# zfkuang/PaletteNeRF

Measured on AMD Instinct MI355X. Metric: rendered_samples_per_sec, higher is better.
Workload: dtype f32 (field: f16x3 split products, fp32 accumulate); 1 GPU; configs[1]: NeRF-synthetic lego geometry (scene S0), -m nerf inference, 800x800, 1 view(s)/step, camera moving (one pose of the path per step); march_mode=native, fused_field=True, field_precision=f16x3, half_tables=False, ray_order=tile8, frames_in_flight=1, gathered_floats_per_ray=0, rccl_ranks=1, parallelism=single GPU

## Files before the change

palettenerf_amd/csrc/field_core.hpp:

```cpp
#pragma once
#include "pnr_common.hpp"
#include "sh_eval.hpp"

namespace pnr {

typedef float f32x16 __attribute__((ext_vector_type(16)));

constexpr int kS0 = 0;
constexpr int kS1 = kS0 + 2 * 16 * 64;
constexpr int kC0 = kS1 + 1 * 32 * 64;
constexpr int kC1 = kC0 + 2 * 16 * 64;
constexpr int kC2 = kC1 + 2 * 32 * 64;
constexpr int kPackedFloats = kC2 + 1 * 32 * 64;

__host__ __device__ constexpr int frag_row(int r, int h) { return (r & 3) + 8 * (r >> 2) + 4 * h; }

__device__ __forceinline__ float select_half(int h, float lower, float upper) {
    const uint32_t m = 0u - (uint32_t)h;
    return __uint_as_float((__float_as_uint(lower) & ~m) | (__float_as_uint(upper) & m));
}

__device__ __forceinline__ f32x16 zero16() {
    f32x16 z;
#pragma unroll
// ... 32 lines not shown
    u32x4 hw, lw;
#pragma unroll
    for (int j = 0; j < 8; j += 2) {
        const h2v hp = {(_Float16)v[j], (_Float16)v[j + 1]};
        const uint32_t hb = __builtin_bit_cast(uint32_t, hp);
        uint32_t lb;
        asm("v_fma_mixlo_f16 %0, %1, -1.0, %2 op_sel_hi:[1,0,0]" : "=v"(lb) : "v"(hb), "v"(v[j]));
        asm("v_fma_mixhi_f16 %0, %1, -1.0, %2 op_sel:[1,0,0] op_sel_hi:[1,0,0]" : "+v"(lb) : "v"(hb), "v"(v[j + 1]));
        hw[j / 2] = hb; lw[j / 2] = lb;
    }
    asm volatile("s_nop 3" : "+v"(lw));
    hi = __builtin_bit_cast(h8, hw);
    lo = __builtin_bit_cast(h8, lw);
}
__device__ __forceinline__ void split_frag(const f32x16& a, int half_idx, h8& hi, h8& lo) {
    float v[8];
#pragma unroll
    for (int j = 0; j < 8; j++) v[j] = a[half_idx * 8 + j];
    split8(v, hi, lo);
}
constexpr int kF16MaxBits = 0x477FE000;
template <bool CHECK> struct SplitWatch;
template <> struct SplitWatch<false> {
    __device__ __forceinline__ void see(const float*) {}
    __device__ __forceinline__ bool overflowed() const { return false; }
};
template <> struct SplitWatch<true> {
    int mx = 0;
    __device__ __forceinline__ void see(const float v[8]) {
#pragma unroll
        for (int j = 0; j < 8; j += 2) mx = max(max(mx, __float_as_int(v[j]) & 0x7fffffff), __float_as_int(v[j + 1]) & 0x7fffffff);
    }
    __device__ __forceinline__ bool overflowed() const { return mx > kF16MaxBits; }
};
template <bool CHECK>
__device__ __forceinline__ void split_frag_w(SplitWatch<CHECK>& sw, const f32x16& a, int half_idx, h8& hi, h8& lo) {
    float v[8];
#pragma unroll
    for (int j = 0; j < 8; j++) v[j] = a[half_idx * 8 + j];
    sw.see(v);
    split8(v, hi, lo);
}

__device__ __forceinline__ f32x16 mma3(f32x16 acc, const unsigned char* __restrict__ wblock, const h8& bhi, const h8& blo, int lane) {
    const h8 ahi = *reinterpret_cast<const h8*>(wblock + lane * 16);
    const h8 alo = *reinterpret_cast<const h8*>(wblock + 1024 + lane * 16);
    acc = __builtin_amdgcn_mfma_f32_32x32x16_f16(alo, bhi, acc, 0, 0, 0);
    acc = __builtin_amdgcn_mfma_f32_32x32x16_f16(ahi, blo, acc, 0, 0, 0);
    acc = __builtin_amdgcn_mfma_f32_32x32x16_f16(ahi, bhi, acc, 0, 0, 0);
    return acc;
}

__device__ __forceinline__ void round8(const float v[8], h8& hi) {
    typedef uint32_t u32x4 __attribute__((ext_vector_type(4)));
    u32x4 hw;
#pragma unroll
    for (int j = 0; j < 8; j += 2) {
        const h2v hp = {(_Float16)v[j], (_Float16)v[j + 1]};
        hw[j / 2] = __builtin_bit_cast(uint32_t, hp);
    }
    hi = __builtin_bit_cast(h8, hw);
}
__device__ __forceinline__ f32x16 mma2(f32x16 acc, const unsigned char* __restrict__ wblock, const h8& bhi, int lane) {
    const h8 ahi = *reinterpret_cast<const h8*>(wblock + lane * 16);
    const h8 alo = *reinterpret_cast<const h8*>(wblock + 1024 + lane * 16);
    acc = __builtin_amdgcn_mfma_f32_32x32x16_f16(alo, bhi, acc, 0, 0, 0);
    acc = __builtin_amdgcn_mfma_f32_32x32x16_f16(ahi, bhi, acc, 0, 0, 0);
    return acc;
}
template <bool LO> __device__ __forceinline__ void splitx(const float v[8], h8& hi, h8& lo) {
    if constexpr (LO) split8(v, hi, lo); else round8(v, hi);
}
template <bool LO> __device__ __forceinline__ f32x16 mmax(f32x16 acc, const unsigned char* __restrict__ wblock, const h8& bhi, const h8& blo, int lane) {
    if constexpr (LO) return mma3(acc, wblock, bhi, blo, lane); else return mma2(acc, wblock, bhi, lane);
}
template <bool LO, bool CHECK>
__device__ __forceinline__ void splitx_frag_w(SplitWatch<CHECK>& sw, const f32x16& a, int half_idx, h8& hi, h8& lo) {
    float v[8];
#pragma unroll
    for (int j = 0; j < 8; j++) v[j] = a[half_idx * 8 + j];
    sw.see(v);
    splitx<LO>(v, hi, lo);
}

template <int PREC> struct BOp;
template <> struct BOp<1> { h8 hi, lo; };
template <> struct BOp<2> { h8 hi; };
template <> struct BOp<0> { float v[8]; };

template <int PREC, bool CHECK = false> __device__ __forceinline__ BOp<PREC> make_op(const float v[8], SplitWatch<CHECK>* sw = nullptr) {
    BOp<PREC> o;
    if constexpr (PREC == 1) { if constexpr (CHECK) sw->see(v); split8(v, o.hi, o.lo); }
    else if constexpr (PREC == 2) { if constexpr (CHECK) sw->see(v); round8(v, o.hi); }
    else {
#pragma unroll
        for (int j = 0; j < 8; j++) o.v[j] = v[j];
    }
    return o;
}
template <int PREC, bool CHECK = false> __device__ __forceinline__ BOp<PREC> frag_op(const f32x16& a, int half_idx, SplitWatch<CHECK>* sw = nullptr) {
    float v[8];
#pragma unroll
    for (int j = 0; j < 8; j++) v[j] = a[half_idx * 8 + j];
    return make_op<PREC, CHECK>(v, sw);
}
template <int PREC> __device__ __forceinline__ f32x16 mma_blk(f32x16 acc, const unsigned char* __restrict__ wblock, const BOp<PREC>& b, int lane) {
    if constexpr (PREC == 1) return mma3(acc, wblock, b.hi, b.lo, lane);
    else if constexpr (PREC == 2) return mma2(acc, wblock, b.hi, lane);
    else {
        const float* w = reinterpret_cast<const float*>(wblock);
#pragma unroll
        for (int j = 0; j < 8; j++) acc = __builtin_amdgcn_mfma_f32_32x32x2f32(w[j * 64 + lane], b.v[j], acc, 0, 0, 0);
        return acc;
    }
}

__device__ __forceinline__ void head3_valu(const unsigned char* __restrict__ vec, const f32x16& u0, const f32x16& u1, float out[3]) {
    typedef float f32x2v __attribute__((ext_vector_type(2)));
    typedef __attribute__((address_space(3))) f32x4 lds_f32x4;
    const lds_f32x4* wv = reinterpret_cast<const lds_f32x4*>(reinterpret_cast<uintptr_t>(vec));
    f32x2v acc[3] = {{0.0f, 0.0f}, {0.0f, 0.0f}, {0.0f, 0.0f}};
#pragma unroll
    for (int t = 0; t < 2; t++)
#pragma unroll
        for (int r4 = 0; r4 < 4; r4++) {
            const f32x16& u = t ? u1 : u0;
            f32x4 ww[3];
#pragma unroll
            for (int o = 0; o < 3; o++) ww[o] = wv[(o * 2 + t) * 4 + r4];
#pragma unroll
            for (int o = 0; o < 3; o++) acc[o] = __builtin_elementwise_fma(f32x2v{ww[o].x, ww[o].y}, f32x2v{u[4 * r4], u[4 * r4 + 1]}, acc[o]);
#pragma unroll
            for (int o = 0; o < 3; o++) acc[o] = __builtin_elementwise_fma(f32x2v{ww[o].z, ww[o].w}, f32x2v{u[4 * r4 + 2], u[4 * r4 + 3]}, acc[o]);
        }
#pragma unroll
    for (int o = 0; o < 3; o++) {
        const float p = acc[o].x + acc[o].y;
        const auto sw2 = __builtin_amdgcn_permlane32_swap(__float_as_uint(p), __float_as_uint(p), false, false);
        out[o] = __uint_as_float(sw2[0]) + __uint_as_float(sw2[1]);
    }
}

constexpr uint32_t kVecHeadHalfBytes = 3 * 2 * 16 * 4;
static __global__ void k_pack_vec_head(const float* __restrict__ w, float* __restrict__ out) {
    const int i = threadIdx.x;
    if (i >= 192) return;
    const int r = i & 15, t = (i >> 4) & 1, o = (i >> 5) % 3, h = i / 96;
    out[i] = w[o * 64 + 32 * t + frag_row(r, h)];
}


struct FieldOut { float sigma_logit, o0, o1, o2; };

__device__ __forceinline__ void load_enc_rows8(const float* __restrict__ enc, size_t level_stride, uint32_t row, bool valid, int h, float x[2][8]) {
    const f32x2* p[8];
    f32x2 v[8];
#pragma unroll
    for (int kb = 0; kb < 2; kb++)
#pragma unroll
        for (int q = 0; q < 4; q++) p[4 * kb + q] = reinterpret_cast<const f32x2*>(enc + ((size_t)(8 * kb + 4 * h + q) * level_stride + row) * 2);
    load8_fresh(p, v);
#pragma unroll
    for (int kb = 0; kb < 2; kb++)
#pragma unroll
        for (int q = 0; q < 4; q++) { x[kb][2 * q] = valid ? v[4 * kb + q].x : 0.0f; x[kb][2 * q + 1] = valid ? v[4 * kb + q].y : 0.0f; }
}
template <bool CHECK, bool LO = true>
__device__ __forceinline__ FieldOut nerf_field_tile_f16x3(const unsigned char* __restrict__ w, int lane, bool valid, const float* __restrict__ enc,
                                                          size_t level_stride, uint32_t row, float dx, float dy, float dz, float enc_scale,
                                                          SplitWatch<CHECK>& sw) {
    const int h = lane >> 5;
    h8 bh[2], bl[2];
    {
        float x[2][8];
        load_enc_rows8(enc, level_stride, row, valid, h, x);
        if (enc_scale != 1.0f) {
#pragma unroll
            for (int j = 0; j < 8; j++) { x[0][j] *= enc_scale; x[1][j] *= enc_scale; }
        }
        sw.see(x[0]); sw.see(x[1]);
        split8(x[0], bh[0], bl[0]);
        split8(x[1], bh[1], bl[1]);
    }
    f32x16 h0 = zero16(), h1 = zero16();
    h0 = mma3(h0, w + 0 * kF16BlockBytes, bh[0], bl[0], lane);
    h0 = mma3(h0, w + 1 * kF16BlockBytes, bh[1], bl[1], lane);
    h1 = mma3(h1, w + 2 * kF16BlockBytes, bh[0], bl[0], lane);
    h1 = mma3(h1, w + 3 * kF16BlockBytes, bh[1], bl[1], lane);
    __builtin_amdgcn_sched_barrier(0);
    h0 = relu16(h0); h1 = relu16(h1);

    f32x16 g = zero16();
#pragma unroll
    for (int kb = 0; kb < 4; kb++) {
        split_frag_w(sw, kb < 2 ? h0 : h1, kb & 1, bh[0], bl[0]);
        g = mma3(g, w + (4 + kb) * kF16BlockBytes, bh[0], bl[0], lane);
    }
    __builtin_amdgcn_sched_barrier(0);
    if (enc_scale != 1.0f) {
        const float inv = 1.0f / enc_scale;
#pragma unroll
        for (int r = 0; r < 8; r++) g[r] *= inv;
    }
    FieldOut out;
    out.sigma_logit = g[0];

    float sh[16];
    sh_eval<4>(dx, dy, dz, sh);
    {
        float v[8];
#pragma unroll
        for (int j = 0; j < 8; j++) v[j] = select_half(h, sh[j], sh[8 + j]);
        splitx<LO>(v, bh[0], bl[0]);
    }
    splitx_frag_w<LO>(sw, g, 0, bh[1], bl[1]);
    f32x16 c0 = zero16(), c1 = zero16();
    c0 = mmax<LO>(c0, w + 8 * kF16BlockBytes, bh[0], bl[0], lane);
    c0 = mmax<LO>(c0, w + 9 * kF16BlockBytes, bh[1], bl[1], lane);
    c1 = mmax<LO>(c1, w + 10 * kF16BlockBytes, bh[0], bl[0], lane);
    c1 = mmax<LO>(c1, w + 11 * kF16BlockBytes, bh[1], bl[1], lane);
    __builtin_amdgcn_sched_barrier(0);
    c0 = relu16(c0); c1 = relu16(c1);

    f32x16 d0 = zero16(), d1 = zero16();
#pragma unroll
    for (int kb = 0; kb < 4; kb++) {
        splitx_frag_w<LO>(sw, kb < 2 ? c0 : c1, kb & 1, bh[0], bl[0]);
        d0 = mmax<LO>(d0, w + (12 + kb) * kF16BlockBytes, bh[0], bl[0], lane);
        d1 = mmax<LO>(d1, w + (16 + kb) * kF16BlockBytes, bh[0], bl[0], lane);
    }
    __builtin_amdgcn_sched_barrier(0);
    d0 = relu16(d0); d1 = relu16(d1);

    float o[3];
    head3_valu(w + 20 * kF16BlockBytes + (uint32_t)h * kVecHeadHalfBytes, d0, d1, o);
    out.o0 = o[0]; out.o1 = o[1]; out.o2 = o[2];
    return out;
}

__device__ __forceinline__ FieldOut nerf_field_tile_f32(const float* __restrict__ w, int lane, bool valid, const float* __restrict__ enc,
                                                        size_t level_stride, uint32_t row, float dx, float dy, float dz) {
    const int h = lane >> 5;
    float x[16];
#pragma unroll
    for (int s = 0; s < 16; s++) x[s] = valid ? enc[((size_t)s * level_stride + row) * 2 + h] : 0.0f;
    f32x16 h0 = zero16(), h1 = zero16();
#pragma unroll
    for (int s = 0; s < 16; s++) {
        h0 = __builtin_amdgcn_mfma_f32_32x32x2f32(w[kS0 + s * 64 + lane], x[s], h0, 0, 0, 0);
        h1 = __builtin_amdgcn_mfma_f32_32x32x2f32(w[kS0 + (16 + s) * 64 + lane], x[s], h1, 0, 0, 0);
    }
    __builtin_amdgcn_sched_barrier(0);
    h0 = relu16(h0); h1 = relu16(h1);
    f32x16 g = zero16();
    g = mma_frag(g, &w[kS1], h0, lane);
    g = mma_frag(g, &w[kS1 + 16 * 64], h1, lane);
    FieldOut out;
    out.sigma_logit = g[0];
    float sh[16];
    sh_eval<4>(dx, dy, dz, sh);
    f32x16 c0 = zero16(), c1 = zero16();
#pragma unroll
    for (int s = 0; s < 8; s++) {
        const float b = select_half(h, sh[s], sh[8 + s]);
        c0 = __builtin_amdgcn_mfma_f32_32x32x2f32(w[kC0 + s * 64 + lane], b, c0, 0, 0, 0);
        c1 = __builtin_amdgcn_mfma_f32_32x32x2f32(w[kC0 + (16 + s) * 64 + lane], b, c1, 0, 0, 0);
    }
    __builtin_amdgcn_sched_barrier(0);
#pragma unroll
    for (int r = 0; r < 8; r++) {
        c0 = __builtin_amdgcn_mfma_f32_32x32x2f32(w[kC0 + (8 + r) * 64 + lane], g[r], c0, 0, 0, 0);
        c1 = __builtin_amdgcn_mfma_f32_32x32x2f32(w[kC0 + (24 + r) * 64 + lane], g[r], c1, 0, 0, 0);
    }
    __builtin_amdgcn_sched_barrier(0);
    c0 = relu16(c0); c1 = relu16(c1);
    f32x16 d0 = zero16(), d1 = zero16();
    d0 = mma_frag(d0, &w[kC1], c0, lane);
    d0 = mma_frag(d0, &w[kC1 + 16 * 64], c1, lane);
    d1 = mma_frag(d1, &w[kC1 + 32 * 64], c0, lane);
    d1 = mma_frag(d1, &w[kC1 + 48 * 64], c1, lane);
    d0 = relu16(d0); d1 = relu16(d1);
    f32x16 o = zero16();
    o = mma_frag(o, &w[kC2], d0, lane);
    o = mma_frag(o, &w[kC2 + 16 * 64], d1, lane);
    out.o0 = o[0]; out.o1 = o[1]; out.o2 = o[2];
    return out;
}

template <int PREC>
__device__ __forceinline__ f32x16 nerf_density_tile(const float* __restrict__ wf, int lane, bool valid, const float* __restrict__ enc, size_t level_stride,
                                                    uint32_t row, float enc_scale = 1.0f) {
    const int h = lane >> 5;
    f32x16 h0 = zero16(), h1 = zero16(), g = zero16();
    if constexpr (PREC == 0) {
        float x[16];
#pragma unroll
        for (int s = 0; s < 16; s++) x[s] = valid ? enc[((size_t)s * level_stride + row) * 2 + h] : 0.0f;
#pragma unroll
        for (int s = 0; s < 16; s++) {
            h0 = __builtin_amdgcn_mfma_f32_32x32x2f32(wf[kS0 + s * 64 + lane], x[s], h0, 0, 0, 0);
            h1 = __builtin_amdgcn_mfma_f32_32x32x2f32(wf[kS0 + (16 + s) * 64 + lane], x[s], h1, 0, 0, 0);
        }
        __builtin_amdgcn_sched_barrier(0);
        h0 = relu16(h0); h1 = relu16(h1);
        g = mma_frag(g, &wf[kS1], h0, lane);
        g = mma_frag(g, &wf[kS1 + 16 * 64], h1, lane);
    } else {
        const unsigned char* w = reinterpret_cast<const unsigned char*>(wf);
        h8 bh[4], bl[4];
        float x[2][8];
        load_enc_rows8(enc, level_stride, row, valid, h, x);
        if (enc_scale != 1.0f) {
#pragma unroll
            for (int j = 0; j < 8; j++) { x[0][j] *= enc_scale; x[1][j] *= enc_scale; }
        }
        split8(x[0], bh[0], bl[0]);
        split8(x[1], bh[1], bl[1]);
        h0 = mma3(h0, w + 0 * kF16BlockBytes, bh[0], bl[0], lane);
        h0 = mma3(h0, w + 1 * kF16BlockBytes, bh[1], bl[1], lane);
        h1 = mma3(h1, w + 2 * kF16BlockBytes, bh[0], bl[0], lane);
        h1 = mma3(h1, w + 3 * kF16BlockBytes, bh[1], bl[1], lane);
        __builtin_amdgcn_sched_barrier(0);
        h0 = relu16(h0); h1 = relu16(h1);
        split_frag(h0, 0, bh[0], bl[0]); split_frag(h0, 1, bh[1], bl[1]);
        split_frag(h1, 0, bh[2], bl[2]); split_frag(h1, 1, bh[3], bl[3]);
#pragma unroll
        for (int kb = 0; kb < 4; kb++) g = mma3(g, w + (4 + kb) * kF16BlockBytes, bh[kb], bl[kb], lane);
        if (enc_scale != 1.0f) {
            const float inv = 1.0f / enc_scale;
#pragma unroll
            for (int r = 0; r < 8; r++) g[r] *= inv;
        }
    }
    return g;
}

template <int PREC, bool CHECK = false>
__device__ __forceinline__ FieldOut nerf_field_tile(const float* __restrict__ w, int lane, bool valid, const float* __restrict__ enc,
                                                    size_t level_stride, uint32_t row, float dx, float dy, float dz, float enc_scale, SplitWatch<CHECK>& sw) {
    if constexpr (PREC == 0) return nerf_field_tile_f32(w, lane, valid, enc, level_stride, row, dx, dy, dz);
    else return nerf_field_tile_f16x3<CHECK, PREC == 1>(reinterpret_cast<const unsigned char*>(w), lane, valid, enc, level_stride, row, dx, dy, dz, enc_scale, sw);
}
template <int PREC>
__device__ __forceinline__ FieldOut nerf_field_tile(const float* __restrict__ w, int lane, bool valid, const float* __restrict__ enc,
                                                    size_t level_stride, uint32_t row, float dx, float dy, float dz, float enc_scale = 1.0f) {
    SplitWatch<false> sw;
    return nerf_field_tile<PREC, false>(w, lane, valid, enc, level_stride, row, dx, dy, dz, enc_scale, sw);
}

}
```

palettenerf_amd/csrc/frame.hip:

```cpp
#include "pnr_common.hpp"
#include "march_core.hpp"
#include "grid_core.hpp"
#include "field_core.hpp"
#include "frame_plan.hpp"
#include <hip/hip_ext.h>
#include <vector>
#include <stdlib.h>

uint64_t pnr_internal_edit_device_bytes();
int pnr_internal_edit_upload(const pnr_palette_edit* edit, void* dst, hipStream_t s);
int pnr_internal_palette_field_forward(const pnr_palette_field_args* a, pnr_stream_t stream, int waves12);

namespace pnr {

struct FrameCtl {
    int32_t n_alive, n_step, step, done;
    int32_t iterations, pad0;
    unsigned long long rendered;
    unsigned long long rows;
    int32_t pad1[6];
};
static_assert(sizeof(FrameCtl) == 64, "FrameCtl layout");

constexpr uint32_t kHdr = 4;
// ... 755 lines not shown
                    step++;
                }
                active = t < r.far && step < n_step;
            }
            emitted += step - (uint32_t)r.step;
            float* pl = h.deltas + ((size_t)row0 + step) * 2;
            for (uint32_t k = step; k < n_step; k++) { pl[0] = 0.0f; pl[1] = 0.0f; pl += 2; }
        }
        __builtin_amdgcn_fence(__ATOMIC_ACQ_REL, "workgroup");
#ifdef PNR_HOSTED_TIMING
        if (timing) {
            uint32_t mp = my_probes;
            for (int off = 32; off > 0; off >>= 1) mp = max(mp, (uint32_t)__shfl_xor((int)mp, off, 64));
            if (lane == 0) { atomicMax(&tm[2], wall_clock64()); atomicMax(&tm[4], (unsigned long long)mp); }
        }
#endif
        const uint32_t nnew = have ? step - (uint32_t)r.step : 0u;
        for (uint32_t k = 0; k < n_step; k++) {
            const bool has_row = k < nnew;
            const unsigned long long m = __ballot(has_row);
            if (m == 0ull) break;
            const uint32_t cnt = (uint32_t)__popcll(m);
            if (has_row) wrows[wave][__popcll(m & ((1ull << lane) - 1ull))] = row0 + (uint32_t)r.step + k;
            wave_lds_sync();
            for (uint32_t pi = (uint32_t)lane; pi < cnt * 16u; pi += PNR_WAVE) {
                const uint32_t b = wrows[wave][pi >> 4], level = pi & 15u;
                LevelCtx lc;
                lc.scale = lv_scale[level]; lc.resolution = lv_res[level]; lc.off0 = lv_off[level]; lc.hashmap_size = lv_size[level];
                lc.kind = 0u;
                for (uint32_t tz = 0; tz < n_tab; tz++) grid_row<KIND, false>(g, lc, level, g.table[tz], g.enc[tz], b);
            }
            wave_lds_sync();
        }
    }
    for (int off = PNR_WAVE / 2; off > 0; off >>= 1) emitted += __shfl_xor(emitted, off, PNR_WAVE);
    if (lane == 0) wemit[wave] = emitted;
    __syncthreads();
    if (threadIdx.x == 0) {
        uint32_t tot = 0;
        for (int wv = 0; wv < (int)(kRayBlock / PNR_WAVE); wv++) tot += wemit[wv];
        h.partials[blockIdx.x] = (int32_t)tot;
#ifdef PNR_HOSTED_TIMING
        if (timing) tm[3] = wall_clock64();
#endif
    }
}

#ifndef PNR_LANE_PAIR_MIN_LEVEL
#define PNR_LANE_PAIR_MIN_LEVEL 8u
#endif
template <int KIND, bool LANE_PAIRS = false>
__device__ __forceinline__ void frame_grid_body(const FrameCtl* __restrict__ ctl, const GridArgs& g, const HostedArgs& h) {
    if (ctl->done) return;
    constexpr uint32_t kLv = KIND == GK_SINGLE ? 2u : 1u;
    constexpr bool kPairs = kLv > 1;
    constexpr uint32_t kNY = 16u / kLv;
    uint32_t bx = blockIdx.x, by = blockIdx.y, bz = blockIdx.z, nbx = gridDim.x;
    if (h.blocks) {
        if (bx < h.blocks) {
            hosted_march_tail<KIND>(ctl, g, h);
            return;
        }
        const uint32_t id = bx - h.blocks, yz = id / h.gx;
        bx = id - yz * h.gx; by = yz % kNY; bz = yz / kNY; nbx = h.gx;
    }
    const uint32_t stride = nbx * 256u;
    const uint32_t rows = (uint32_t)ctl->n_alive * (uint32_t)ctl->n_step;
    const uint32_t level = 15u - by;
#ifdef PNR_HOSTED_TIMING
    const bool timing = ctl->iterations == g_hosted_timing_iter && (bx & 15u) == 0 && bx < 2048u && bz == 0;
    unsigned long long* tmm = g_hosted_timing + 8 + 8 * 256 + 2 * (level * 128 + (bx >> 4));
    if (timing && threadIdx.x == 0) tmm[0] = wall_clock64();
#endif
    const LevelCtx lc = level_ctx(g, level);
    [[maybe_unused]] const LevelCtx lc2 = level_ctx(g, kPairs ? by : level);
    const void* table = g.table[KIND == GK_SINGLE ? bz : 0];
    float* enc0 = g.enc[KIND == GK_SINGLE ? bz : 0];
    bool paired = false;
    if constexpr (LANE_PAIRS) {
        if (level >= PNR_LANE_PAIR_MIN_LEVEL) {
            paired = true;
            if constexpr (kPairs) {
                const LevelCtx lcs[2] = {lc, lc2};
                const uint32_t levels[2] = {level, by};
                grid_pair_rows<KIND, 2>(g, lcs, levels, table, enc0, h.rowflag, bx * 256u + threadIdx.x, stride, rows);
            } else {
                const LevelCtx lcs[1] = {lc};
                const uint32_t levels[1] = {level};
                grid_pair_rows<KIND, 1>(g, lcs, levels, table, enc0, h.rowflag, bx * 256u + threadIdx.x, stride, rows);
            }
        }
    }
    if (!paired)
    for (uint32_t b = bx * 256u + threadIdx.x; b < rows; b += stride) {
        const float d0 = g.deltas[(size_t)b * 2];
        const uint32_t fl = h.rowflag ? h.rowflag[b] : 0u;
        if (d0 == 0.0f || fl) continue;
        grid_row<KIND>(g, lc, level, table, enc0, b);
        if constexpr (kPairs) grid_row<KIND>(g, lc2, by, table, enc0, b);
    }
#ifdef PNR_HOSTED_TIMING
    if (timing && threadIdx.x == 0) { asm volatile("s_waitcnt vmcnt(0)" ::: "memory"); tmm[1] = wall_clock64(); }
#endif
}

#ifndef PNR_GRID_WAVES
#define PNR_GRID_WAVES 8
#endif
#ifndef PNR_GRID_WAVES_SINGLE
#define PNR_GRID_WAVES_SINGLE 7
#endif
#define PNR_GRID_KERNEL(NAME, KIND, WAVES, ...)                                                                                              \
    __global__ void __launch_bounds__(256) __attribute__((amdgpu_waves_per_eu(WAVES))) NAME(const FrameCtl* __restrict__ ctl, GridArgs g, HostedArgs h) { \
        frame_grid_body<KIND, ##__VA_ARGS__>(ctl, g, h);                                                                                     \
    }
PNR_GRID_KERNEL(k_frame_grid, GK_SINGLE, PNR_GRID_WAVES_SINGLE)
PNR_GRID_KERNEL(k_frame_grid_lp, GK_SINGLE, PNR_GRID_WAVES_SINGLE, true)
PNR_GRID_KERNEL(k_frame_grid_pair, GK_PAIR, PNR_GRID_WAVES)
PNR_GRID_KERNEL(k_frame_grid_triple, GK_TRIPLE, PNR_GRID_WAVES)
PNR_GRID_KERNEL(k_frame_grid_h1, GK_HALF1, PNR_GRID_WAVES)
PNR_GRID_KERNEL(k_frame_grid_h2, GK_HALF2, PNR_GRID_WAVES)
PNR_GRID_KERNEL(k_frame_grid_h3, GK_HALF3, PNR_GRID_WAVES)
#undef PNR_GRID_KERNEL

__global__ void __launch_bounds__(256) k_interleave_tables(const float2* __restrict__ a, const float2* __restrict__ b, uint64_t rows,
                                                           float4* __restrict__ out) {
    const uint64_t i = (uint64_t)blockIdx.x * 256 + threadIdx.x;
    if (i < rows) { const float2 u = a[i], v = b[i]; out[i] = make_float4(u.x, u.y, v.x, v.y); }
}
__global__ void __launch_bounds__(256) k_interleave_tables3(const float2* __restrict__ a, const float2* __restrict__ b, const float2* __restrict__ c,
                                                            uint64_t rows, float4* __restrict__ out) {
    const uint64_t i = (uint64_t)blockIdx.x * 256 + threadIdx.x;
    if (i < rows) {
        const float2 u = a[i], v = b[i], t = c[i];
        out[2 * i] = make_float4(u.x, u.y, v.x, v.y);
        out[2 * i + 1] = make_float4(t.x, t.y, 0.0f, 0.0f);
    }
}
__global__ void __launch_bounds__(256) k_interleave_tables3_half(const float2* __restrict__ a, const float2* __restrict__ b, const float2* __restrict__ c,
                                                                 uint64_t rows, uint4* __restrict__ out) {
    const uint64_t i = (uint64_t)blockIdx.x * 256 + threadIdx.x;
    if (i < rows) {
        const float2 u = a[i], v = b[i], t = c[i];
        const __half h[8] = {__float2half(u.x), __float2half(u.y), __float2half(v.x), __float2half(v.y), __float2half(t.x), __float2half(t.y),
                             __float2half(0.0f), __float2half(0.0f)};
        uint4 row;
        __builtin_memcpy(&row, h, sizeof(row));
        out[i] = row;
    }
}

constexpr int kFieldThreads = 512;
template <int PREC, bool CHECK>
__global__ void __launch_bounds__(kFieldThreads) k_frame_field(const FrameCtl* __restrict__ ctl, const float* __restrict__ enc, uint32_t level_stride,
                                                               const float* __restrict__ dirs, const float* __restrict__ deltas,
                                                               const float* __restrict__ packed, float density_scale, float enc_scale, float* __restrict__ sigmas,
                                                               float* __restrict__ rgbs, int fuse_mode, float T_thresh, int32_t* __restrict__ rays_alive,
                                                               float* __restrict__ rays_t, float* __restrict__ weights_sum, float* __restrict__ depth,
                                                               float* __restrict__ image, int32_t* __restrict__ scratch, int32_t* __restrict__ counts_cur) {
    if (ctl->done) return;
    const uint32_t n_step = (uint32_t)ctl->n_step;
    const uint32_t B = (uint32_t)ctl->n_alive * n_step;
    const bool fuse = fuse_mode && n_step == 1;
    const bool fuse_rays = fuse_mode == 2 && n_step > 1;
    const uint32_t rpw = fuse_rays ? (32u / n_step) * n_step : 32u;
    const uint32_t rpt = rpw * (kFieldThreads / PNR_WAVE);
    const uint32_t ntiles = (B + rpt - 1) / rpt;
    if (blockIdx.x >= ntiles) return;
    __shared__ float w[kPackedFloats];
    __shared__ int wsum[kFieldThreads / PNR_WAVE];
    for (int i = threadIdx.x * 4; i < kPackedFloats; i += kFieldThreads * 4) lds_copy16(&packed[i], &w[i]);
    bool weights_ready = false;
    const int lane = threadIdx.x & 63, wave = threadIdx.x >> 6, h = lane >> 5;
    const uint32_t l = (uint32_t)lane & 31u;
    for (uint32_t tile = blockIdx.x; tile < ntiles; tile += gridDim.x) {
        const uint32_t n = tile * rpt + wave * rpw + l;
        const bool mine = l < rpw && n < B;
        const float dl0 = mine ? deltas[(size_t)n * 2] : 0.0f;
        const bool valid = mine && dl0 != 0.0f;
        FieldOut o = {0.0f, 0.0f, 0.0f, 0.0f};
        const uint32_t nc = n < B ? n : (B - 1);
        float dx = 0.0f, dy = 0.0f, dz = 0.0f;
        if (valid) { dx = dirs[(size_t)nc * 3]; dy = dirs[(size_t)nc * 3 + 1]; dz = dirs[(size_t)nc * 3 + 2]; }
        if (!weights_ready) { lds_copy_wait(); __syncthreads(); weights_ready = true; }
        if (__any(valid)) {
            SplitWatch<CHECK> sw;
            o = nerf_field_tile<PREC, CHECK>(w, lane, valid, enc, level_stride, nc, dx, dy, dz, enc_scale, sw);
            if constexpr (CHECK) { if (sw.overflowed()) scratch[1] = 1; }
        }
        float sigma = 0.0f, cr = 0.0f, cg = 0.0f, cb = 0.0f;
        if (valid && h == 0) {
            sigma = density_scale * __expf(o.sigma_logit);
            cr = __frcp_rn(1.0f + __expf(-o.o0));
            cg = __frcp_rn(1.0f + __expf(-o.o1));
            cb = __frcp_rn(1.0f + __expf(-o.o2));
            if (!fuse && !fuse_rays) {
                sigmas[n] = sigma;
                rgbs[(size_t)n * 3] = cr; rgbs[(size_t)n * 3 + 1] = cg; rgbs[(size_t)n * 3 + 2] = cb;
            }
        }
        if (fuse) {
            int keep = 0;
            if (h == 0 && n < B) {
                const int index = rays_alive[n];
                float ws = weights_sum[index], t = rays_t[index], d = depth[index];
                float r = image[index * 3], g = image[index * 3 + 1], b = image[index * 3 + 2];
                bool stepped = false;
                if (dl0 != 0.0f) {
                    const float alpha = 1.0f - __expf(-sigma * dl0);
                    const float T = 1.0f - ws;
                    const float wgt = alpha * T;
                    ws += wgt;
                    t += deltas[(size_t)n * 2 + 1];
                    d = fmaf(wgt, t, d);
                    r = fmaf(wgt, cr, r); g = fmaf(wgt, cg, g); b = fmaf(wgt, cb, b);
                    stepped = !(T < T_thresh);
                }
                if (!stepped) rays_alive[n] = -1; else { rays_t[index] = t; keep = 1; }
                weights_sum[index] = ws; depth[index] = d;
                image[index * 3] = r; image[index * 3 + 1] = g; image[index * 3 + 2] = b;
            }
            const unsigned long long m = __ballot(keep);
            if (lane == 0) wsum[wave] = __popcll(m);
            __syncthreads();
            if (threadIdx.x == 0) {
                int tot = 0;
                for (int wv = 0; wv < kFieldThreads / (int)PNR_WAVE; wv++) tot += wsum[wv];
                counts_cur[tile] = tot;
            }
            __syncthreads();
        } else if (fuse_rays) {
            const float dl1 = (valid && h == 0) ? deltas[(size_t)n * 2 + 1] : 0.0f;
            const bool leader = h == 0 && mine && (l % n_step) == 0;
            const uint32_t slot = n / n_step;
            int index = 0;
            float ws = 0.0f, t = 0.0f, d = 0.0f, r = 0.0f, g = 0.0f, b = 0.0f;
            if (leader) {
                index = rays_alive[slot];
                ws = weights_sum[index]; t = rays_t[index]; d = depth[index];
                r = image[index * 3]; g = image[index * 3 + 1]; b = image[index * 3 + 2];
            }
            uint32_t step = 0;
            bool running = leader;
            for (uint32_t k = 0; k < n_step; k++) {
                const int src = lane + (int)k;
                const float s_k = __shfl(sigma, src), a_k = __shfl(dl0, src), b_k = __shfl(dl1, src);
                const float r_k = __shfl(cr, src), g_k = __shfl(cg, src), c_k = __shfl(cb, src);
                if (running) {
                    if (a_k == 0.0f) running = false;
                    else {
                        const float alpha = 1.0f - __expf(-s_k * a_k);
                        const float T = 1.0f - ws;
                        const float wgt = alpha * T;
                        ws += wgt;
                        t += b_k;
                        d = fmaf(wgt, t, d);
                        r = fmaf(wgt, r_k, r); g = fmaf(wgt, g_k, g); b = fmaf(wgt, c_k, b);
                        if (T < T_thresh) running = false; else step++;
                    }
                }
            }
            int keep = 0;
            if (leader) {
                if (step < n_step) rays_alive[slot] = -1; else { rays_t[index] = t; keep = 1; }
                weights_sum[index] = ws; depth[index] = d;
                image[index * 3] = r; image[index * 3 + 1] = g; image[index * 3 + 2] = b;
            }
            const unsigned long long km = __ballot(keep);
            if (km != 0ull) {
                const uint32_t c0 = ((tile * rpt + wave * rpw) / n_step) >> 8;
                const unsigned long long k0 = __ballot(keep && (slot >> 8) == c0);
                if (lane == 0) {
                    if (k0) atomicAdd(&counts_cur[c0], __popcll(k0));
                    if (km & ~k0) atomicAdd(&counts_cur[c0 + 1], __popcll(km & ~k0));
                }
            }
        }
    }
}

__global__ void __launch_bounds__(kRayBlock) k_frame_composite(const FrameCtl* __restrict__ ctl, float T_thresh, int32_t* __restrict__ rays_alive,
                                                               float* __restrict__ rays_t, const float* __restrict__ sigmas,
                                                               const float* __restrict__ rgbs, const float* __restrict__ deltas,
                                                               float* __restrict__ weights_sum, float* __restrict__ depth, float* __restrict__ image,
                                                               int32_t* __restrict__ counts_cur, const float* __restrict__ aux, float* __restrict__ aux_map,
                                                               uint32_t aux_stride, int aux_done_when_one_step, int all_done_when_one_step) {
    if (ctl->done) return;
    const uint32_t n_alive = (uint32_t)ctl->n_alive, n_step = (uint32_t)ctl->n_step;
    if (all_done_when_one_step && n_step == 1) return;
    const uint32_t nchunks = (n_alive + kRayBlock - 1) / kRayBlock;
    __shared__ int wsum[kRayBlock / PNR_WAVE];
    for (uint32_t chunk = blockIdx.x; chunk < nchunks; chunk += gridDim.x) {
        if (aux && !(aux_done_when_one_step && n_step <= 8 && (32 % n_step) == 0)) {
            const uint32_t nq = aux_stride / 4, rays_per_pass = kRayBlock / nq;
            const uint32_t slot = threadIdx.x / nq, q = threadIdx.x - slot * nq;
            for (uint32_t r = slot; r < kRayBlock && slot < rays_per_pass; r += rays_per_pass) {
                const uint32_t n = chunk * kRayBlock + r;
                if (n >= n_alive) continue;
                const int index = rays_alive[n];
                const float* s = sigmas + (size_t)n * n_step;
                const float* in = aux + (size_t)n * n_step * aux_stride + q * 4;
                const float* dl = deltas + (size_t)n * n_step * 2;
                float4* out = reinterpret_cast<float4*>(aux_map + (size_t)index * aux_stride) + q;
                float4 acc = *out;
                float ws = weights_sum[index];
                for (uint32_t step = 0; step < n_step; step++) {
                    if (dl[0] == 0) break;
                    const float alpha = 1.0f - __expf(-s[0] * dl[0]);
                    const float T = 1.0f - ws;
                    const float wgt = alpha * T;
                    ws += wgt;
                    const float4 v = *reinterpret_cast<const float4*>(in);
                    acc.x = fmaf(wgt, v.x, acc.x); acc.y = fmaf(wgt, v.y, acc.y); acc.z = fmaf(wgt, v.z, acc.z); acc.w = fmaf(wgt, v.w, acc.w);
                    if (T < T_thresh) break;
                    s++; in += aux_stride; dl += 2;
                }
                *out = acc;
            }
            __syncthreads();
        }
        const uint32_t n = chunk * kRayBlock + threadIdx.x;
        int keep = 0;
        if (n < n_alive) {
            const int index = rays_alive[n];
            const float ws0 = weights_sum[index];
            const float* s = sigmas + (size_t)n * n_step;
            const float* c = rgbs + (size_t)n * n_step * 3;
            const float* dl = deltas + (size_t)n * n_step * 2;
            float t = rays_t[index], ws = ws0, d = depth[index];
            float r = image[index * 3], g = image[index * 3 + 1], b = image[index * 3 + 2];
            uint32_t step = 0;
            while (step < n_step) {
                if (dl[0] == 0) break;
                const float alpha = 1.0f - __expf(-s[0] * dl[0]);
                const float T = 1.0f - ws;
                const float wgt = alpha * T;
                ws += wgt;
                t += dl[1];
                d = fmaf(wgt, t, d);
                r = fmaf(wgt, c[0], r); g = fmaf(wgt, c[1], g); b = fmaf(wgt, c[2], b);
                if (T < T_thresh) break;
                s++; c += 3; dl += 2; step++;
            }
            if (step < n_step) rays_alive[n] = -1; else { rays_t[index] = t; keep = 1; }
            weights_sum[index] = ws; depth[index] = d;
            image[index * 3] = r; image[index * 3 + 1] = g; image[index * 3 + 2] = b;
        }
        const unsigned long long m = __ballot(keep);
        if ((threadIdx.x & (PNR_WAVE - 1)) == 0) wsum[threadIdx.x / PNR_WAVE] = __popcll(m);
        __syncthreads();
        if (threadIdx.x == 0) {
            int tot = 0;
            for (int wv = 0; wv < (int)(kRayBlock / PNR_WAVE); wv++) tot += wsum[wv];
            counts_cur[chunk] = tot;
        }
        __syncthreads();
    }
}

struct FrameWorkspace {
    FrameCtl* ctl;
    int32_t* alive[2];
    float *rays_t, *xyzs, *dirs, *deltas, *enc, *sigmas, *rgbs;
    float *enc_pal, *enc_clip, *aux;
    void* edit;
    float *s_o, *s_d, *s_noise, *s_far, *s_ws, *s_depth, *s_image, *s_aux;
    int32_t* scratch;
    int32_t* partials[2];
    HostedConst* hosted;
    int32_t* qctr;
    StragglerRec* qrecs;
    uint8_t* rowflag;
    uint64_t bytes;
};
static FrameWorkspace carve(void* base, uint32_t N, uint32_t aux_stride = 0, bool with_clip = false) {
    FrameWorkspace w;
    uint64_t off = 0;
    auto take = [&](uint64_t nbytes) { char* p = base ? static_cast<char*>(base) + off : nullptr; off += align256(nbytes); return p; };
    const uint64_t n = N ? N : 1;
    w.ctl = reinterpret_cast<FrameCtl*>(take(2 * sizeof(FrameCtl)));
    w.alive[0] = reinterpret_cast<int32_t*>(take(n * 4));
    w.alive[1] = reinterpret_cast<int32_t*>(take(n * 4));
    w.rays_t = reinterpret_cast<float*>(take(n * 4));
    w.xyzs = reinterpret_cast<float*>(take(n * 12));
    w.dirs = reinterpret_cast<float*>(take(n * 12));
    w.deltas = reinterpret_cast<float*>(take(n * 8));
    w.enc = reinterpret_cast<float*>(take(n * 16 * 2 * 4));
    w.sigmas = reinterpret_cast<float*>(take(n * 4));
    w.rgbs = reinterpret_cast<float*>(take(n * 12));
    w.scratch = reinterpret_cast<int32_t*>(take((kHdr + 2 * (n / kRayBlock + 2)) * 4));
    w.partials[0] = reinterpret_cast<int32_t*>(take((kMaxMarchBlocks + kHostedBlocks) * 4));
    w.partials[1] = reinterpret_cast<int32_t*>(take((kMaxMarchBlocks + kHostedBlocks) * 4));
    w.enc_pal = w.enc_clip = w.aux = nullptr;
    w.edit = nullptr;
    if (aux_stride) {
        w.edit = take(pnr_internal_edit_device_bytes());
        w.enc_pal = reinterpret_cast<float*>(take(n * 16 * 2 * 4));
        if (with_clip) w.enc_clip = reinterpret_cast<float*>(take(n * 16 * 2 * 4));
        w.aux = reinterpret_cast<float*>(take(n * aux_stride * 4));
    }
    w.s_o = reinterpret_cast<float*>(take(n * 12)); w.s_d = reinterpret_cast<float*>(take(n * 12));
    w.s_noise = reinterpret_cast<float*>(take(n * 4)); w.s_far = reinterpret_cast<float*>(take(n * 4));
    w.s_ws = reinterpret_cast<float*>(take(n * 4)); w.s_depth = reinterpret_cast<float*>(take(n * 4));
    w.s_image = reinterpret_cast<float*>(take(n * 12));
    w.s_aux = aux_stride ? reinterpret_cast<float*>(take(n * aux_stride * 4)) : nullptr;
    w.hosted = reinterpret_cast<HostedConst*>(take(sizeof(HostedConst)));
    w.qctr = reinterpret_cast<int32_t*>(take(2 * kQueueCtrs * 4));
    w.qrecs = reinterpret_cast<StragglerRec*>(take(n * sizeof(StragglerRec)));
    w.rowflag = reinterpret_cast<uint8_t*>(take(n));
    w.bytes = off;
    return w;
}

struct FrameOpts {
#define PNR_OPTION(name, def, set, env, what)
#define PNR_FRAME_OPTION(name, def, set, env, what) int name;
#include "options.def"
};
static FrameOpts frame_opts_now() {
    FrameOpts o;
#define PNR_OPTION(name, def, set, env, what)
#define PNR_FRAME_OPTION(name, def, set, env, what) o.name = g_opt_##name;
#include "options.def"
// ... 396 lines not shown
```

palettenerf_amd/csrc/frame_plan.hpp:

```cpp
#pragma once
#include <stdint.h>

namespace pnr {

constexpr uint32_t kRayBlock = 256;
#ifndef PNR_MAX_MARCH_BLOCKS
#define PNR_MAX_MARCH_BLOCKS 4096
#endif
constexpr uint32_t kMaxMarchBlocks = PNR_MAX_MARCH_BLOCKS;
constexpr uint32_t kResidentMarchBlocks = 1280;

inline uint64_t align256(uint64_t v) { return (v + 255) & ~uint64_t(255); }
inline uint32_t plan_cdiv(uint32_t a, uint32_t b) { return (a + b - 1) / b; }
inline uint32_t plan_min(uint32_t a, uint32_t b) { return a < b ? a : b; }

inline uint32_t first_chunk(uint32_t predicted, uint32_t margin) {
    return predicted ? plan_min(predicted + 1u + margin, 1024u) : 8u;
}
inline uint32_t next_chunk(uint32_t chunk, uint32_t& looks, uint32_t predicted) {
    if (looks == 0) chunk = predicted ? 4u : 8u;
    if (++looks >= 4 && chunk < 64) chunk *= 2;
    return chunk;
}
inline uint32_t rows_upper_bound(uint32_t alive_ub, uint32_t N) { return (uint64_t)alive_ub * 8 < N ? alive_ub * 8 : N; }
inline uint32_t lookup_blocks(uint32_t rows_ub) { return plan_cdiv(rows_ub, 256); }
inline uint32_t lookup_blocks_capped(uint32_t rows_ub) { return plan_min(lookup_blocks(rows_ub), 1024u); }
inline uint32_t field_blocks(uint32_t rows_ub) { return plan_min(lookup_blocks(rows_ub), 512u); }
inline uint32_t march_budget(bool hosted, int iter, int budget_first, int budget_later) { return hosted ? (uint32_t)(iter == 0 ? budget_first : budget_later) : 0u; }
inline int march_mode(uint32_t budget) { return budget ? 2 : 1; }
inline uint32_t march_blocks(uint32_t alive_ub, int mode, int march_blocks_option) {
    const uint32_t ray_blocks = plan_cdiv(alive_ub, kRayBlock);
    uint32_t cap = kMaxMarchBlocks;
    if (mode == 2) {
        if (march_blocks_option > 0 && march_blocks_option < 65536) cap = plan_min((uint32_t)march_blocks_option, kMaxMarchBlocks);
        else if (ray_blocks >= 2 * kResidentMarchBlocks) cap = kResidentMarchBlocks;
    }
    return plan_min(ray_blocks, cap);
}

}
```

Baseline: 3.073 billion samples/s.

## Prefetch field encodings before weight sync and drop per-tile block barriers

The field kernel now gives each wave its own tile of rays through a new wave-tile mapping instead of block-wide tiles. For the f16x3 path, the hash-encoding rows, directions and ray index are loaded before the first weight-LDS wait, so those global loads overlap the weight copy. The two __syncthreads per tile used for the per-block alive count are replaced by per-wave atomics into counts_cur indexed by wt>>3. A waves_per_eu hint of 4 is added for the f16x3 path, which caps registers per thread. That cap risks spills, and the changed counts indexing must still match what the consumer expects.

Measured after the change: 3.182 billion samples/s (median of 6 runs). 3.5% higher.

```diff
diff --git a/palettenerf_amd/csrc/field_core.hpp b/palettenerf_amd/csrc/field_core.hpp
--- a/palettenerf_amd/csrc/field_core.hpp
+++ b/palettenerf_amd/csrc/field_core.hpp
@@ -208,28 +208,31 @@
 
 struct FieldOut { float sigma_logit, o0, o1, o2; };
 
-__device__ __forceinline__ void load_enc_rows8(const float* __restrict__ enc, size_t level_stride, uint32_t row, bool valid, int h, float x[2][8]) {
+__device__ __forceinline__ void load_enc_raw8(const float* __restrict__ enc, size_t level_stride, uint32_t row, int h, f32x2 (&v)[8]) {
     const f32x2* p[8];
-    f32x2 v[8];
 #pragma unroll
     for (int kb = 0; kb < 2; kb++)
 #pragma unroll
         for (int q = 0; q < 4; q++) p[4 * kb + q] = reinterpret_cast<const f32x2*>(enc + ((size_t)(8 * kb + 4 * h + q) * level_stride + row) * 2);
     load8_fresh(p, v);
+}
+__device__ __forceinline__ void enc_rows8_of(const f32x2 (&v)[8], bool valid, float x[2][8]) {
 #pragma unroll
     for (int kb = 0; kb < 2; kb++)
 #pragma unroll
         for (int q = 0; q < 4; q++) { x[kb][2 * q] = valid ? v[4 * kb + q].x : 0.0f; x[kb][2 * q + 1] = valid ? v[4 * kb + q].y : 0.0f; }
 }
+__device__ __forceinline__ void load_enc_rows8(const float* __restrict__ enc, size_t level_stride, uint32_t row, bool valid, int h, float x[2][8]) {
+    f32x2 v[8];
+    load_enc_raw8(enc, level_stride, row, h, v);
+    enc_rows8_of(v, valid, x);
+}
 template <bool CHECK, bool LO = true>
-__device__ __forceinline__ FieldOut nerf_field_tile_f16x3(const unsigned char* __restrict__ w, int lane, bool valid, const float* __restrict__ enc,
-                                                          size_t level_stride, uint32_t row, float dx, float dy, float dz, float enc_scale,
-                                                          SplitWatch<CHECK>& sw) {
+__device__ __forceinline__ FieldOut nerf_field_tile_f16x3_rows(const unsigned char* __restrict__ w, int lane, float x[2][8], float dx, float dy, float dz,
+                                                               float enc_scale, SplitWatch<CHECK>& sw) {
     const int h = lane >> 5;
     h8 bh[2], bl[2];
     {
-        float x[2][8];
-        load_enc_rows8(enc, level_stride, row, valid, h, x);
         if (enc_scale != 1.0f) {
 #pragma unroll
             for (int j = 0; j < 8; j++) { x[0][j] *= enc_scale; x[1][j] *= enc_scale; }
@@ -292,6 +295,14 @@
     head3_valu(w + 20 * kF16BlockBytes + (uint32_t)h * kVecHeadHalfBytes, d0, d1, o);
     out.o0 = o[0]; out.o1 = o[1]; out.o2 = o[2];
     return out;
+}
+template <bool CHECK, bool LO = true>
+__device__ __forceinline__ FieldOut nerf_field_tile_f16x3(const unsigned char* __restrict__ w, int lane, bool valid, const float* __restrict__ enc,
+                                                          size_t level_stride, uint32_t row, float dx, float dy, float dz, float enc_scale,
+                                                          SplitWatch<CHECK>& sw) {
+    float x[2][8];
+    load_enc_rows8(enc, level_stride, row, valid, lane >> 5, x);
+    return nerf_field_tile_f16x3_rows<CHECK, LO>(w, lane, x, dx, dy, dz, enc_scale, sw);
 }
 
 __device__ __forceinline__ FieldOut nerf_field_tile_f32(const float* __restrict__ w, int lane, bool valid, const float* __restrict__ enc,
diff --git a/palettenerf_amd/csrc/frame.hip b/palettenerf_amd/csrc/frame.hip
--- a/palettenerf_amd/csrc/frame.hip
+++ b/palettenerf_amd/csrc/frame.hip
@@ -931,7 +931,8 @@
 
 constexpr int kFieldThreads = 512;
 template <int PREC, bool CHECK>
-__global__ void __launch_bounds__(kFieldThreads) k_frame_field(const FrameCtl* __restrict__ ctl, const float* __restrict__ enc, uint32_t level_stride,
+__global__ void __launch_bounds__(kFieldThreads) __attribute__((amdgpu_waves_per_eu((PREC != 0 && !CHECK) ? 4 : 2)))
+k_frame_field(const FrameCtl* __restrict__ ctl, const float* __restrict__ enc, uint32_t level_stride,
                                                                const float* __restrict__ dirs, const float* __restrict__ deltas,
                                                                const float* __restrict__ packed, float density_scale, float enc_scale, float* __restrict__ sigmas,
                                                                float* __restrict__ rgbs, int fuse_mode, float T_thresh, int32_t* __restrict__ rays_alive,
@@ -943,28 +944,51 @@
     const bool fuse = fuse_mode && n_step == 1;
     const bool fuse_rays = fuse_mode == 2 && n_step > 1;
     const uint32_t rpw = fuse_rays ? (32u / n_step) * n_step : 32u;
-    const uint32_t rpt = rpw * (kFieldThreads / PNR_WAVE);
-    const uint32_t ntiles = (B + rpt - 1) / rpt;
-    if (blockIdx.x >= ntiles) return;
+    const uint32_t nwt = (B + rpw - 1) / rpw;
+    constexpr uint32_t kWaves = kFieldThreads / PNR_WAVE;
+    if (field_wave_tile(0, 0, blockIdx.x, gridDim.x, kWaves) >= nwt) return;
     __shared__ float w[kPackedFloats];
-    __shared__ int wsum[kFieldThreads / PNR_WAVE];
     for (int i = threadIdx.x * 4; i < kPackedFloats; i += kFieldThreads * 4) lds_copy16(&packed[i], &w[i]);
-    bool weights_ready = false;
-    const int lane = threadIdx.x & 63, wave = threadIdx.x >> 6, h = lane >> 5;
+    const int lane = threadIdx.x & 63, h = lane >> 5;
+    const uint32_t wave = (uint32_t)__builtin_amdgcn_readfirstlane((int)(threadIdx.x >> 6));
     const uint32_t l = (uint32_t)lane & 31u;
-    for (uint32_t tile = blockIdx.x; tile < ntiles; tile += gridDim.x) {
-        const uint32_t n = tile * rpt + wave * rpw + l;
-        const bool mine = l < rpw && n < B;
-        const float dl0 = mine ? deltas[(size_t)n * 2] : 0.0f;
+    for (uint32_t it = 0;; it++) {
+        const uint32_t wt = field_wave_tile(it, wave, blockIdx.x, gridDim.x, kWaves);
+        const bool have = wt < nwt;
+        if (it != 0 && !have) break;
+        const uint32_t n = wt * rpw + l;
+        const bool mine = have && l < rpw && n < B;
+        f32x2 dl = {0.0f, 0.0f};
+        if (mine) dl = *reinterpret_cast<const f32x2*>(deltas + (size_t)n * 2);
+        int index_early = 0;
+        if (fuse && mine && h == 0) index_early = rays_alive[n];
+        const float dl0 = dl.x;
         const bool valid = mine && dl0 != 0.0f;
         FieldOut o = {0.0f, 0.0f, 0.0f, 0.0f};
         const uint32_t nc = n < B ? n : (B - 1);
         float dx = 0.0f, dy = 0.0f, dz = 0.0f;
-        if (valid) { dx = dirs[(size_t)nc * 3]; dy = dirs[(size_t)nc * 3 + 1]; dz = dirs[(size_t)nc * 3 + 2]; }
-        if (!weights_ready) { lds_copy_wait(); __syncthreads(); weights_ready = true; }
+        constexpr bool kEarlyEnc = PREC != 0 && !CHECK;
+        [[maybe_unused]] f32x2 ev[8];
+        if constexpr (kEarlyEnc) {
+            if (have) {
+                load_enc_raw8(enc, level_stride, nc, h, ev);
+                dx = dirs[(size_t)nc * 3]; dy = dirs[(size_t)nc * 3 + 1]; dz = dirs[(size_t)nc * 3 + 2];
+            }
+            dx = valid ? dx : 0.0f; dy = valid ? dy : 0.0f; dz = valid ? dz : 0.0f;
+        } else {
+            if (valid) { dx = dirs[(size_t)nc * 3]; dy = dirs[(size_t)nc * 3 + 1]; dz = dirs[(size_t)nc * 3 + 2]; }
+        }
+        if (it == 0) { lds_copy_wait(); __syncthreads(); }
+        if (!have) break;
         if (__any(valid)) {
             SplitWatch<CHECK> sw;
-            o = nerf_field_tile<PREC, CHECK>(w, lane, valid, enc, level_stride, nc, dx, dy, dz, enc_scale, sw);
+            if constexpr (kEarlyEnc) {
+                float x[2][8];
+                enc_rows8_of(ev, valid, x);
+                o = nerf_field_tile_f16x3_rows<CHECK, PREC == 1>(reinterpret_cast<const unsigned char*>(w), lane, x, dx, dy, dz, enc_scale, sw);
+            } else {
+                o = nerf_field_tile<PREC, CHECK>(w, lane, valid, enc, level_stride, nc, dx, dy, dz, enc_scale, sw);
+            }
             if constexpr (CHECK) { if (sw.overflowed()) scratch[1] = 1; }
         }
         float sigma = 0.0f, cr = 0.0f, cg = 0.0f, cb = 0.0f;
@@ -981,7 +1005,7 @@
         if (fuse) {
             int keep = 0;
             if (h == 0 && n < B) {
-                const int index = rays_alive[n];
+                const int index = index_early;
                 float ws = weights_sum[index], t = rays_t[index], d = depth[index];
                 float r = image[index * 3], g = image[index * 3 + 1], b = image[index * 3 + 2];
                 bool stepped = false;
@@ -990,7 +1014,7 @@
                     const float T = 1.0f - ws;
                     const float wgt = alpha * T;
                     ws += wgt;
-                    t += deltas[(size_t)n * 2 + 1];
+                    t += dl.y;
                     d = fmaf(wgt, t, d);
                     r = fmaf(wgt, cr, r); g = fmaf(wgt, cg, g); b = fmaf(wgt, cb, b);
                     stepped = !(T < T_thresh);
@@ -1000,16 +1024,9 @@
                 image[index * 3] = r; image[index * 3 + 1] = g; image[index * 3 + 2] = b;
             }
             const unsigned long long m = __ballot(keep);
-            if (lane == 0) wsum[wave] = __popcll(m);
-            __syncthreads();
-            if (threadIdx.x == 0) {
-                int tot = 0;
-                for (int wv = 0; wv < kFieldThreads / (int)PNR_WAVE; wv++) tot += wsum[wv];
-                counts_cur[tile] = tot;
-            }
-            __syncthreads();
+            if (m != 0ull && lane == 0) atomicAdd(&counts_cur[wt >> 3], __popcll(m));
         } else if (fuse_rays) {
-            const float dl1 = (valid && h == 0) ? deltas[(size_t)n * 2 + 1] : 0.0f;
+            const float dl1 = (valid && h == 0) ? dl.y : 0.0f;
             const bool leader = h == 0 && mine && (l % n_step) == 0;
             const uint32_t slot = n / n_step;
             int index = 0;
@@ -1047,7 +1064,7 @@
             }
             const unsigned long long km = __ballot(keep);
             if (km != 0ull) {
-                const uint32_t c0 = ((tile * rpt + wave * rpw) / n_step) >> 8;
+                const uint32_t c0 = ((wt * rpw) / n_step) >> 8;
                 const unsigned long long k0 = __ballot(keep && (slot >> 8) == c0);
                 if (lane == 0) {
                     if (k0) atomicAdd(&counts_cur[c0], __popcll(k0));
diff --git a/palettenerf_amd/csrc/frame_plan.hpp b/palettenerf_amd/csrc/frame_plan.hpp
--- a/palettenerf_amd/csrc/frame_plan.hpp
+++ b/palettenerf_amd/csrc/frame_plan.hpp
@@ -26,6 +26,9 @@
 inline uint32_t lookup_blocks(uint32_t rows_ub) { return plan_cdiv(rows_ub, 256); }
 inline uint32_t lookup_blocks_capped(uint32_t rows_ub) { return plan_min(lookup_blocks(rows_ub), 1024u); }
 inline uint32_t field_blocks(uint32_t rows_ub) { return plan_min(lookup_blocks(rows_ub), 512u); }
+constexpr uint32_t field_wave_tile(uint32_t it, uint32_t wave, uint32_t block, uint32_t grid, uint32_t waves) {
+    return it * grid * waves + (wave / 4u) * (grid * 4u) + block * 4u + (wave % 4u);
+}
 inline uint32_t march_budget(bool hosted, int iter, int budget_first, int budget_later) { return hosted ? (uint32_t)(iter == 0 ? budget_first : budget_later) : 0u; }
 inline int march_mode(uint32_t budget) { return budget ? 2 : 1; }
 inline uint32_t march_blocks(uint32_t alive_ub, int mode, int march_blocks_option) {
```
